# ChristophReich1996/Multi-StyleGAN

Hardware: AMD Instinct MI355X
Metric: training images/sec (G+D step, 256^2, seq=3x2ch) (higher is better)
Workload: dtype bf16

## Files before the change

multi_stylegan_amd/csrc/conv_dispatch.h:

```cpp
#pragma once
#include "msg_common.h"

struct ConvProblem {
    int dtype;
    int split;
    int B, IH, IW, Cx, Ck, OH, OW, N, ldy;
    int kh, kw, stride, pad, in_up, pixel_shuffle;
    long long w_batch_stride;

    bool per_sample() const { return w_batch_stride != 0; }
    int samples() const { return per_sample() ? B : 1; }
    long long mtot() const { return per_sample() ? (long long)OH * OW : (long long)B * OH * OW; }
    int esz() const { return dtype == MSG_BF16 ? 2 : 4; }
    long long x_bstride() const { return (long long)IH * IW * Cx; }
    long long y_bstride() const { return (pixel_shuffle ? 4ll : 1ll) * OH * OW * ldy; }
    long long x_bytes() const { return (long long)(per_sample() ? 1 : B) * IH * IW * Cx * esz(); }
    long long w_bytes() const { return (long long)N * kh * kw * Ck * esz(); }
    bool fits31() const { return x_bytes() < 0x7ffffff0ll && w_bytes() < 0x7ffffff0ll; }
};

enum ConvKernel {
    CONV_THIN_N, CONV_THIN_K,
    CONV_UPCONV,
    CONV_ROW3, CONV_ROW3N,
    CONV_PP,
    CONV_DMA, CONV_REG, CONV_REG_LEAN, CONV_REG_SPLIT
};

struct ConvPlan {
    ConvKernel kernel;
    int tile_m, tile_n;
    bool supported;
};

inline int conv_act_mode(const ActEpilogue* act) { return act ? act->enabled : 0; }

template <typename P>
inline void conv_fill_common(P& p, const ConvProblem& q, const ActEpilogue* act) {
    p.B = q.B; p.IH = q.IH; p.IW = q.IW; p.Cx = q.Cx; p.Ck = q.Ck; p.OH = q.OH; p.OW = q.OW; p.N = q.N; p.ldy = q.ldy;
    p.per_sample = q.per_sample();
    if (act) p.act = *act;
    p.x_bstride = q.x_bstride();
    p.w_bstride = q.w_batch_stride;
    p.y_bstride = q.y_bstride();
    p.Mtot = (int)q.mtot();
}
template <typename P>
inline void conv_fill_taps(P& p, const ConvProblem& q) {
    p.kh = q.kh; p.kw = q.kw; p.stride = q.stride; p.pad = q.pad; p.in_up = q.in_up; p.pixel_shuffle = q.pixel_shuffle;
}

ConvPlan conv_fprop_select(const ConvProblem& q, const ActEpilogue* act, bool has_bias);

bool conv_thin_eligible(const ConvProblem& q, const ActEpilogue* act, ConvPlan* plan);
void conv_thin_launch(const ConvProblem& q, const ConvPlan& plan, const void* x, const void* w, const float* bias, void* y,
                      const ActEpilogue* act, void* stream);
bool conv_upconv_eligible(const ConvProblem& q, const ActEpilogue* act, bool has_bias, ConvPlan* plan);
void conv_upconv_launch(const ConvProblem& q, const ConvPlan& plan, const void* x, const void* w, void* y, void* stream);
bool conv_row3_eligible(const ConvProblem& q, const ActEpilogue* act, bool has_bias, ConvPlan* plan);
void conv_row3_launch(const ConvProblem& q, const ConvPlan& plan, const void* x, const void* w, const float* bias, void* y,
                      const ActEpilogue* act, void* stream);
bool conv_pp_eligible(const ConvProblem& q, ConvPlan* plan);
void conv_pp_launch(const ConvProblem& q, const ConvPlan& plan, const void* x, const void* w, const float* bias, void* y,
                    const ActEpilogue* act, void* stream);

struct WgradProblem {
    int dtype;
    int split;
    int B, IH, IW, Cx, I, OH, OW, ldgy, O, ldgw;
    int kh, kw, stride, pad, pixel_shuffle;
    int per_sample, k_chunks, oi_major;
    float gain;
};

int conv_wgrad_row3_try(const WgradProblem& q, const void* gy, const void* x, float* gw, float* ws, long long ws_floats,
                        int plan_only, long long* need, void* stream);
extern "C" int msg_wgrad_reduce_launch(const float* ws, float* gw, long long slab, int n_out, int chunks, int O, int taps,
                                       int I, int ldgw, int oi_major, void* stream);
```

multi_stylegan_amd/csrc/conv_fprop.hip:

```cpp
#include "conv_dispatch.h"
#include <stdlib.h>

typedef __bf16 bf16v8 __attribute__((ext_vector_type(8)));
typedef const __attribute__((address_space(1))) char* gptr_t;
typedef const __attribute__((address_space(1))) u32x4* gvec_t;
typedef __attribute__((address_space(3))) char* lds_t;

struct ConvParams {
    int B, IH, IW, Cx, Ck, OH, OW, N, ldy;
    int kh, kw, stride, pad, in_up, pixel_shuffle, per_sample;
    long long x_bstride, w_bstride, y_bstride;
    int Mtot, n_chunks, n_iters, m_tiles, n_tiles;
    ActEpilogue act;
};

constexpr int BM = 128, BN = 128, ROWB = 128;
constexpr int STAGE_BYTES = (BM + BN) * ROWB;
__device__ __attribute__((aligned(256))) unsigned int g_zero_page[16384];

__device__ __forceinline__ int swz(int row, int slot) { return row * ROWB + ((slot ^ ((row >> 1) & 7)) << 4); }

template <int SPLIT>
__device__ __forceinline__ void split_park(const u32x4& raw, char* dst) {
    uint2 pl[3];
#pragma unroll
    for (int h = 0; h < 2; ++h) {
        const float x0 = __uint_as_float(raw[2 * h]), x1 = __uint_as_float(raw[2 * h + 1]);
        const unsigned hp = (unsigned)f2bf(x0) | ((unsigned)f2bf(x1) << 16);
        const float r0 = x0 - __uint_as_float(hp << 16), r1 = x1 - __uint_as_float(hp & 0xffff0000u);
        const unsigned mp = (unsigned)f2bf(r0) | ((unsigned)f2bf(r1) << 16);
        (h ? pl[0].y : pl[0].x) = hp;
        (h ? pl[1].y : pl[1].x) = mp;
        if constexpr (SPLIT == 3) {
            const float q0 = r0 - __uint_as_float(mp << 16), q1 = r1 - __uint_as_float(mp & 0xffff0000u);
            (h ? pl[2].y : pl[2].x) = (unsigned)f2bf(q0) | ((unsigned)f2bf(q1) << 16);
        }
    }
#pragma unroll
    for (int p = 0; p < SPLIT; ++p) *reinterpret_cast<uint2*>(dst + p * 64) = pl[p];
}

template <typename T, bool DMA, int LEAN = 0, int SPLIT = 0>
__global__ __launch_bounds__(256, LEAN ? LEAN : 2) void conv_fprop_kernel(const T* __restrict__ x, const T* __restrict__ w,
                                                            T* __restrict__ y, const float* __restrict__ bias,
                                                            ConvParams p) {
    constexpr int VEC = 16 / sizeof(T);
    constexpr int BKE = ROWB / sizeof(T);
    static_assert(!LEAN || (!DMA && sizeof(T) == 2), "lean variant: bf16, register staging");
    static_assert(SPLIT == 0 || sizeof(T) == 4, "split-bf16 products are a mode of the fp32-storage kernel");
    static_assert(SPLIT == 0 || !DMA, "the split planes are written from the staging registers");
    constexpr int SROW = SPLIT ? SPLIT * 64 + 16 : ROWB;
    constexpr int STAGE = SPLIT ? (BM + BN) * SROW : STAGE_BYTES;
    constexpr bool ONE_STAGE = LEAN != 0 || SPLIT == 3;
    constexpr int SMEM_BYTES = ONE_STAGE ? (STAGE > 65536 || sizeof(T) == 2 ? STAGE : 65536) : 2 * STAGE;
    __shared__ __attribute__((aligned(16))) char smem[SMEM_BYTES];

    const int tid = threadIdx.x, lane = tid & 63, wid = tid >> 6;
    const int wm = wid >> 1, wn = wid & 1;
    const int lr = lane & 31, lh = lane >> 5;
    const unsigned L = xcd_remap(blockIdx.x, gridDim.x);
    const int n0 = (int)(L % p.n_tiles) * BN;
    const int m0 = (int)(L / p.n_tiles) * BM;
    const int bz = blockIdx.z;

    const int wid_u = __builtin_amdgcn_readfirstlane(wid);
    const int slot_phys = tid & 7;
    int row_of[4];
#pragma unroll
    for (int j = 0; j < 4; ++j) row_of[j] = DMA ? (wid * 32 + 8 * j + (lane >> 3)) : ((tid >> 3) + 32 * j);
    const int slot = DMA ? 0 : slot_phys;
    int a_ih0[4], a_iw0[4];
    long long a_boff[4];
    int a_slot[4];
    bool a_ok[4];
    const int ohw = p.OH * p.OW;
#pragma unroll
    for (int j = 0; j < 4; ++j) {
        const int m = m0 + row_of[j];
        const int slot_j = DMA ? (slot_phys ^ ((row_of[j] >> 1) & 7)) : slot_phys;
        a_ok[j] = m < p.Mtot;
        const int mm = a_ok[j] ? m : 0;
        const int b = p.per_sample ? bz : mm / ohw;
        const int pix = p.per_sample ? mm : mm - b * ohw;
        const int oh = pix / p.OW, ow = pix - oh * p.OW;
        a_ih0[j] = oh * p.stride - p.pad;
        a_iw0[j] = ow * p.stride - p.pad;
        a_boff[j] = ((long long)((DMA && p.per_sample) ? 0 : b) * p.x_bstride + slot_j * VEC +
                     ((long long)a_ih0[j] * p.IW + a_iw0[j]) * p.Cx) * (long long)sizeof(T);
        a_slot[j] = slot_j;
    }
    const int taps = p.kh * p.kw;
    const gptr_t xbase = (gptr_t)x;
    const gptr_t zbase = (gptr_t)g_zero_page;
    const long long zoff = slot_phys * 16;
    gptr_t pa[4];
    gptr_t pb[4];
    {
        const gptr_t wb = (gptr_t)w + (p.per_sample ? (long long)bz * p.w_bstride : 0) * (long long)sizeof(T);
#pragma unroll
        for (int j = 0; j < 4; ++j) {
            const int n = n0 + row_of[j];
            const bool ok = n < p.N;
            pb[j] = (ok ? wb : zbase) + (ok ? ((long long)n * taps * p.Ck + a_slot[j] * VEC) * (long long)sizeof(T) : zoff);
            pa[j] = zbase;
        }
    }
    msg_desc_t d_x = {0, 0, 0, 0}, d_w = {0, 0, 0, 0};
    unsigned lds0 = 0;
    int va[4] = {MSG_DMA_OOB, MSG_DMA_OOB, MSG_DMA_OOB, MSG_DMA_OOB}, vb[4] = {MSG_DMA_OOB, MSG_DMA_OOB, MSG_DMA_OOB, MSG_DMA_OOB};
    if constexpr (DMA) {
        d_x = msg_make_desc((const char*)x + (p.per_sample ? (long long)bz * p.x_bstride * (long long)sizeof(T) : 0));
        d_w = msg_make_desc((const char*)w + (p.per_sample ? (long long)bz * p.w_bstride * (long long)sizeof(T) : 0));
        lds0 = (unsigned)(unsigned long long)(lds_t)smem;
#pragma unroll
        for (int j = 0; j < 4; ++j) {
            const int n = n0 + row_of[j];
            vb[j] = n < p.N ? (int)(((long long)n * taps * p.Ck + a_slot[j] * VEC) * (long long)sizeof(T)) : MSG_DMA_OOB;
        }
    }
    const bool ragged = (p.Cx % BKE) != 0;
    int ld_tap = -1, ld_chunk = p.n_chunks - 1;
    int kh_ = 0, kw_ = -1;
    int st_off[4];
#pragma unroll
    for (int j = 0; j < 4; ++j) st_off[j] = swz(row_of[j], a_slot[j]);

    f32x16 acc[2][2];
#pragma unroll
    for (int i = 0; i < 2; ++i)
#pragma unroll
        for (int j = 0; j < 2; ++j)
#pragma unroll
            for (int e = 0; e < 16; ++e) acc[i][j][e] = 0.f;

    u32x4 ra[4], rb[4];
    int dma_stage = 0;
    auto load_next = [&]() __attribute__((always_inline)) {
        if (++ld_chunk == p.n_chunks) {
            ld_chunk = 0;
            ++ld_tap;
            if (++kw_ == p.kw) { kw_ = 0; ++kh_; }
            if (p.in_up == 1) {
                const long long tap_off = ((long long)kh_ * p.IW + kw_) * p.Cx * (long long)sizeof(T);
#pragma unroll
                for (int j = 0; j < 4; ++j) {
                    const bool ok = a_ok[j] & ((unsigned)(a_ih0[j] + kh_) < (unsigned)p.IH) &
                                    ((unsigned)(a_iw0[j] + kw_) < (unsigned)p.IW);
                    pa[j] = (ok ? xbase : zbase) + (ok ? a_boff[j] + tap_off : zoff);
                    if constexpr (DMA) va[j] = ok ? (int)(a_boff[j] + tap_off) : MSG_DMA_OOB;
                }
            } else {
#pragma unroll
                for (int j = 0; j < 4; ++j) {
                    const int ih = a_ih0[j] + kh_, iw = a_iw0[j] + kw_;
                    bool ok = a_ok[j] & (ih >= 0) & (iw >= 0) & (ih % p.in_up == 0) & (iw % p.in_up == 0);
                    const int ihs = ih / p.in_up, iws = iw / p.in_up;
                    ok = ok & (ihs < p.IH) & (iws < p.IW);
                    const long long off = a_boff[j] + ((long long)(ihs - a_ih0[j]) * p.IW + (iws - a_iw0[j])) * p.Cx * (long long)sizeof(T);
                    pa[j] = (ok ? xbase : zbase) + (ok ? off : zoff);
                    if constexpr (DMA) va[j] = ok ? (int)off : MSG_DMA_OOB;
                }
            }
        }
#pragma unroll
        for (int j = 0; j < 4; ++j) {
            const bool c_bad = ragged && (ld_chunk * BKE + a_slot[j] * VEC + VEC > p.Cx);
            gptr_t a_addr = pa[j];
            if (c_bad) a_addr = zbase + zoff;
            if constexpr (DMA) {
                const unsigned la = lds0 + dma_stage * STAGE + (wid_u * 32 + 8 * j) * ROWB;
                msg_dma16(d_x, la, c_bad ? MSG_DMA_OOB : va[j], ld_chunk * ROWB);
                msg_dma16(d_w, la + BM * ROWB, vb[j], (ld_tap * p.n_chunks + ld_chunk) * ROWB);
            } else {
                ra[j] = *(gvec_t)a_addr;
                rb[j] = *(gvec_t)pb[j];
            }
            pa[j] += ROWB;
            pb[j] += ROWB;
        }
    };
    auto park = [&](int stage) __attribute__((always_inline)) {
        char* sa = smem + stage * STAGE;
        if constexpr (SPLIT != 0) {
            char* sb = sa + BM * SROW;
#pragma unroll
            for (int j = 0; j < 4; ++j) {
                split_park<SPLIT>(ra[j], sa + row_of[j] * SROW + slot_phys * 8);
                split_park<SPLIT>(rb[j], sb + row_of[j] * SROW + slot_phys * 8);
            }
            return;
        }
        char* sb = sa + BM * ROWB;
#pragma unroll
        for (int j = 0; j < 4; ++j) {
            *reinterpret_cast<u32x4*>(sa + st_off[j]) = ra[j];
            *reinterpret_cast<u32x4*>(sb + st_off[j]) = rb[j];
        }
    };
    auto mma_step = [&](const char* sa) __attribute__((always_inline)) {
        const char* sb = sa + BM * ROWB;
        if constexpr (sizeof(T) == 2) {
            bf16v8 fa[2][2], fb[2][2];
#pragma unroll
            for (int t = 0; t < 2; ++t) {
                fa[0][t] = *reinterpret_cast<const bf16v8*>(sa + swz(wm * 64 + t * 32 + lr, lh));
                fb[0][t] = *reinterpret_cast<const bf16v8*>(sb + swz(wn * 64 + t * 32 + lr, lh));
            }
#pragma unroll
            for (int kk = 0; kk < 4; ++kk) {
                if (kk + 1 < 4) {
#pragma unroll
                    for (int t = 0; t < 2; ++t) {
                        fa[(kk + 1) & 1][t] = *reinterpret_cast<const bf16v8*>(sa + swz(wm * 64 + t * 32 + lr, 2 * (kk + 1) + lh));
                        fb[(kk + 1) & 1][t] = *reinterpret_cast<const bf16v8*>(sb + swz(wn * 64 + t * 32 + lr, 2 * (kk + 1) + lh));
                    }
                }
#pragma unroll
                for (int i = 0; i < 2; ++i)
#pragma unroll
                    for (int j = 0; j < 2; ++j)
                        acc[i][j] = __builtin_amdgcn_mfma_f32_32x32x16_bf16(fb[kk & 1][j], fa[kk & 1][i], acc[i][j], 0, 0, 0);
            }
            __builtin_amdgcn_sched_group_barrier(0x100, 8, 0);
            __builtin_amdgcn_sched_group_barrier(0x008, 4, 0);
            __builtin_amdgcn_sched_group_barrier(0x100, 4, 0);
            __builtin_amdgcn_sched_group_barrier(0x008, 4, 0);
            __builtin_amdgcn_sched_group_barrier(0x100, 4, 0);
            __builtin_amdgcn_sched_group_barrier(0x008, 8, 0);
        } else if constexpr (SPLIT != 0) {
            const char* sbs = sa + BM * SROW;
#pragma unroll
            for (int sstep = 0; sstep < 2; ++sstep) {
                bf16v8 af[SPLIT][2], bf[SPLIT][2];
#pragma unroll
                for (int t = 0; t < 2; ++t)
#pragma unroll
                    for (int pl = 0; pl < SPLIT; ++pl) {
                        af[pl][t] = *reinterpret_cast<const bf16v8*>(sa + (wm * 64 + t * 32 + lr) * SROW + pl * 64 + (2 * sstep + lh) * 16);
                        bf[pl][t] = *reinterpret_cast<const bf16v8*>(sbs + (wn * 64 + t * 32 + lr) * SROW + pl * 64 + (2 * sstep + lh) * 16);
                    }
#pragma unroll
                for (int i = 0; i < 2; ++i)
#pragma unroll
                    for (int j = 0; j < 2; ++j) {
#pragma unroll
                        for (int order = SPLIT - 1; order >= 0; --order)
#pragma unroll
                            for (int pa = 0; pa <= order; ++pa)
                                acc[i][j] = __builtin_amdgcn_mfma_f32_32x32x16_bf16(bf[order - pa][j], af[pa][i], acc[i][j], 0, 0, 0);
                    }
            }
        } else {
#pragma unroll
            for (int q = 0; q < 4; ++q) {
                f32x4 fa[2], fb[2];
#pragma unroll
                for (int t = 0; t < 2; ++t) {
                    fa[t] = *reinterpret_cast<const f32x4*>(sa + swz(wm * 64 + t * 32 + lr, 4 * lh + q));
                    fb[t] = *reinterpret_cast<const f32x4*>(sb + swz(wn * 64 + t * 32 + lr, 4 * lh + q));
                }
#pragma unroll
                for (int e = 0; e < 4; ++e)
#pragma unroll
                    for (int i = 0; i < 2; ++i)
#pragma unroll
                        for (int j = 0; j < 2; ++j)
                            acc[i][j] = __builtin_amdgcn_mfma_f32_32x32x2f32(fb[j][e], fa[i][e], acc[i][j], 0, 0, 0);
            }
        }
    };
    if constexpr (ONE_STAGE) {
        load_next();
        for (int it = 0; it < p.n_iters; ++it) {
            if (it) __syncthreads();
            park(0);
            if (it + 1 < p.n_iters) load_next();
            __syncthreads();
            mma_step(smem);
        }
    } else {
        if constexpr (DMA) {
            dma_stage = 0;
            load_next();
        } else {
            load_next();
            park(0);
            if (p.n_iters > 1) load_next();
        }
        for (int it = 0; it < p.n_iters; ++it) {
            if constexpr (DMA) asm volatile("s_waitcnt vmcnt(0)" ::: "memory");
            __syncthreads();
            if constexpr (DMA) {
                if (it + 1 < p.n_iters) { dma_stage = (it + 1) & 1; load_next(); }
            } else {
                if (it + 1 < p.n_iters) park((it + 1) & 1);
                if (it + 2 < p.n_iters) load_next();
            }
            mma_step(smem + (it & 1) * STAGE);
        }
    }
    if constexpr (DMA) asm volatile("s_waitcnt vmcnt(0)" ::: "memory");
    __syncthreads();

    constexpr int PITCH = 64 * sizeof(T);
    constexpr int UNITB = 4 * sizeof(T);
    char* ep = smem + wid * (64 * PITCH);
#pragma unroll
    for (int j = 0; j < 2; ++j)
#pragma unroll
        for (int g = 0; g < 4; ++g) {
            const int unit = 8 * j + 2 * g + lh;
            float bv[4] = {0.f, 0.f, 0.f, 0.f};
            if (bias) {
                const int nb = n0 + wn * 64 + 4 * unit;
#pragma unroll
                for (int e = 0; e < 4; ++e) bv[e] = nb + e < p.N ? bias[nb + e] : 0.f;
            }
#pragma unroll
            for (int i = 0; i < 2; ++i) {
                const int row = i * 32 + lr;
                char* dstl = ep + row * PITCH + ((unit ^ (row & 15)) * UNITB);
                if constexpr (sizeof(T) == 2) {
                    uint2 pk;
                    pk.x = (unsigned)f2bf(acc[i][j][4 * g + 0] + bv[0]) | ((unsigned)f2bf(acc[i][j][4 * g + 1] + bv[1]) << 16);
                    pk.y = (unsigned)f2bf(acc[i][j][4 * g + 2] + bv[2]) | ((unsigned)f2bf(acc[i][j][4 * g + 3] + bv[3]) << 16);
                    *reinterpret_cast<uint2*>(dstl) = pk;
                } else {
                    *reinterpret_cast<f32x4*>(dstl) = f32x4{acc[i][j][4 * g + 0] + bv[0], acc[i][j][4 * g + 1] + bv[1],
                                                            acc[i][j][4 * g + 2] + bv[2], acc[i][j][4 * g + 3] + bv[3]};
                }
            }
        }
    constexpr int LPR = 64 / VEC;
    constexpr int RPP = 64 / LPR;
    constexpr int NPASS = 64 / RPP;
    const int er = lane / LPR, ec = (lane % LPR) * VEC;
    const int n = n0 + wn * 64 + ec;
    int nn = n, q = 0;
    if (p.pixel_shuffle) { const int oc = p.N >> 2; q = n / oc; nn = n - q * oc; }
    const int lim = p.pixel_shuffle ? (p.N >> 2) - nn : p.N - n;
    const bool n_ok = n < p.N;
    int gp[NPASS];
    float a_bias[VEC], a_noise[NPASS];
    {
        const int m_first = min(m0 + wm * 64 + er, p.Mtot - 1);
        int b = p.per_sample ? bz : m_first / ohw;
        const int pix0 = p.per_sample ? m_first : m_first - b * ohw;
        int oh = pix0 / p.OW, ow = pix0 - oh * p.OW;
        const bool want_noise = p.act.enabled == 1 && p.act.noise;
        const float nw = want_noise ? p.act.noise_w[0] : 0.f;
        if (p.act.enabled == 1) {
#pragma unroll
            for (int e = 0; e < VEC; ++e) a_bias[e] = (p.act.bias && n + e < p.N) ? p.act.bias[n + e] : 0.f;
        }
#pragma unroll
        for (int pass = 0; pass < NPASS; ++pass) {
            const bool ok = m0 + wm * 64 + pass * RPP + er < p.Mtot;
            const int pix = oh * p.OW + ow;
            const int g = p.pixel_shuffle ? ((b * 2 * p.OH + 2 * oh + (q >> 1)) * (2 * p.OW) + 2 * ow + (q & 1))
                                          : b * ohw + pix;
            gp[pass] = ok ? g : -1;
            a_noise[pass] = (want_noise && ok) ? nw * p.act.noise[(long long)(p.act.noise_batch == 1 ? 0 : b) * ohw + pix] : 0.f;
            ow += RPP;
            while (ow >= p.OW) { ow -= p.OW; ++oh; }
            if (!p.per_sample) while (oh >= p.OH) { oh -= p.OH; ++b; }
        }
    }
    __syncthreads();
    u32x4 v[NPASS];
#pragma unroll
    for (int pass = 0; pass < NPASS; ++pass) {
        const int row = pass * RPP + er;
        if constexpr (sizeof(T) == 2)
            v[pass] = *reinterpret_cast<const u32x4*>(ep + row * PITCH + (((lane & 7) ^ ((row & 15) >> 1)) << 4));
        else
            v[pass] = *reinterpret_cast<const u32x4*>(ep + row * PITCH + (((lane & 15) ^ (row & 15)) << 4));
    }
    if constexpr (sizeof(T) == 2) {
        if (er & 1) {
#pragma unroll
            for (int pass = 0; pass < NPASS; ++pass) v[pass] = u32x4{v[pass][2], v[pass][3], v[pass][0], v[pass][1]};
        }
    }
    if (p.act.enabled == 1) {
#pragma unroll
        for (int pass = 0; pass < NPASS; ++pass) v[pass] = act_epilogue_apply<T>(v[pass], a_bias, a_noise[pass], p.act.alpha, p.act.scale);
    } else if (p.act.enabled == 2) {
        const T* rbase = reinterpret_cast<const T*>(p.act.residual) + (n_ok ? n : 0);
        u32x4 r[NPASS];
#pragma unroll
        for (int pass = 0; pass < NPASS; ++pass)
            r[pass] = *reinterpret_cast<const u32x4*>(rbase + (long long)max(gp[pass], 0) * p.act.res_ld);
#pragma unroll
        for (int pass = 0; pass < NPASS; ++pass) v[pass] = residual_epilogue_apply<T>(v[pass], r[pass], p.act.res_gain);
    }
    T* ybase = y + (p.pixel_shuffle ? nn : n);
    if (n_ok && lim >= VEC) {
#pragma unroll
        for (int pass = 0; pass < NPASS; ++pass)
            if (gp[pass] >= 0) *reinterpret_cast<u32x4*>(ybase + (long long)gp[pass] * p.ldy) = v[pass];
    } else if (n_ok) {
#pragma unroll
        for (int pass = 0; pass < NPASS; ++pass) {
            if (gp[pass] < 0) continue;
            T tmp[VEC];
            *reinterpret_cast<u32x4*>(tmp) = v[pass];
            T* dst = ybase + (long long)gp[pass] * p.ldy;
            for (int e = 0; e < lim; ++e) dst[e] = tmp[e];
        }
    }
}

static ConvPlan conv_generic_select(const ConvProblem& q) {
    const int n_iters = q.kh * q.kw * (q.Ck / (ROWB / q.esz()));
    static const int variant = msg_tunable("MSG_CONV_VARIANT", 0);
    const bool dma = q.fits31() && (variant == 1 || (variant == 0 && n_iters >= 8));
    static const int lean_max = msg_tunable("MSG_CONV_LEAN", 4);
    ConvPlan plan{CONV_REG, BM, BN, true};
    if (q.split) plan.kernel = CONV_REG_SPLIT;
    else if (dma) plan.kernel = CONV_DMA;
    else if (q.dtype == MSG_BF16 && n_iters <= lean_max) plan.kernel = CONV_REG_LEAN;
    const long long mtot = q.mtot(), blocks = ((mtot + BM - 1) / BM) * ((q.N + BN - 1) / BN);
    plan.supported = mtot < (1ll << 31) && blocks < (1ll << 31) &&
                     (long long)(n_iters + 1) * ROWB + 128 <= 65536;
    return plan;
}

static void conv_generic_launch(const ConvProblem& q, const ConvPlan& plan, const void* x, const void* w, const float* bias, void* y,
                                const ActEpilogue* act, void* stream) {
    ConvParams p{};
    conv_fill_common(p, q, act);
    conv_fill_taps(p, q);
    p.n_chunks = q.Ck / (ROWB / q.esz());
    p.n_iters = q.kh * q.kw * p.n_chunks;
    p.m_tiles = (int)((q.mtot() + BM - 1) / BM);
    p.n_tiles = (q.N + BN - 1) / BN;
    dim3 grid((unsigned)((long long)p.m_tiles * p.n_tiles), 1, q.samples());
#define GENERIC(T, ...) hipLaunchKernelGGL((conv_fprop_kernel<T, __VA_ARGS__>), grid, dim3(256), 0, (hipStream_t)stream, \
                                           (const T*)x, (const T*)w, (T*)y, bias, p)
    const bool bf16 = q.dtype == MSG_BF16;
    if (bf16 && plan.kernel == CONV_REG_LEAN) GENERIC(bf16_t, false, 3);
    else if (bf16 && plan.kernel == CONV_DMA) GENERIC(bf16_t, true);
    else if (bf16) GENERIC(bf16_t, false);
    else if (plan.kernel == CONV_REG_SPLIT) GENERIC(float, false, 0, 3);
    else if (plan.kernel == CONV_DMA) GENERIC(float, true);
    else GENERIC(float, false);
#undef GENERIC
}

ConvPlan conv_fprop_select(const ConvProblem& q, const ActEpilogue* act, bool has_bias) {
    ConvPlan plan;
    if (conv_thin_eligible(q, act, &plan)) return plan;
    if (conv_upconv_eligible(q, act, has_bias, &plan)) return plan;
    if (conv_row3_eligible(q, act, has_bias, &plan)) return plan;
    if (conv_pp_eligible(q, &plan)) return plan;
    return conv_generic_select(q);
}

static ConvProblem conv_problem(int dtype, int B, int IH, int IW, int Cx, int Ck, int OH, int OW, int N, int ldy,
                                int kh, int kw, int stride, int pad, int in_up, int pixel_shuffle, long long w_batch_stride) {
    const int split = dtype == MSG_F32_SPLIT ? 3 : 0;
    return ConvProblem{split ? (int)MSG_F32 : dtype, split, B, IH, IW, Cx, Ck, OH, OW, N, ldy, kh, kw, stride, pad, in_up, pixel_shuffle,
                       w_batch_stride};
}
static ConvProblem conv_query_problem(int dtype, int B, int IH, int IW, int Cx, int Ck, int OH, int OW, int N, int kh, int kw,
                                      long long w_batch_stride) {
    return conv_problem(dtype, B, IH, IW, Cx, Ck, OH, OW, N, N <= 8 ? 8 : (N + 7) / 8 * 8, kh, kw, 1, kh / 2, 1, 0, w_batch_stride);
}

extern "C" int msg_conv2d_fprop_plan(int dtype, int B, int IH, int IW, int Cx, int Ck, int OH, int OW, int N,
                                     int kh, int kw, long long w_batch_stride) {
    switch (conv_fprop_select(conv_query_problem(dtype, B, IH, IW, Cx, Ck, OH, OW, N, kh, kw, w_batch_stride), nullptr, false).kernel) {
        case CONV_THIN_N: case CONV_THIN_K: return MSG_PLAN_THIN;
        case CONV_ROW3: return MSG_PLAN_ROW3;
        case CONV_ROW3N: return MSG_PLAN_ROW3N;
        case CONV_PP: return MSG_PLAN_PP;
        case CONV_UPCONV: return MSG_PLAN_PP;
        case CONV_DMA: return MSG_PLAN_DMA;
        default: return MSG_PLAN_REG;
    }
}

static int conv2d_fprop_impl(const void* x, const void* w, const float* bias, void* y, const ConvProblem& q,
                             const ActEpilogue& act, void* stream, const ConvPlan* selected = nullptr);

extern "C" int msg_conv2d_fprop(const void* x, const void* w, const float* bias, void* y, int dtype,
                                int B, int IH, int IW, int Cx, int Ck, int OH, int OW, int N, int ldy,
                                int kh, int kw, int stride, int pad, int in_up, int pixel_shuffle,
                                long long w_batch_stride, void* stream) {
    ActEpilogue act{};
    return conv2d_fprop_impl(x, w, bias, y, conv_problem(dtype, B, IH, IW, Cx, Ck, OH, OW, N, ldy, kh, kw, stride, pad, in_up,
                                                         pixel_shuffle, w_batch_stride), act, stream);
}

static bool is_row3(const ConvPlan& plan) { return plan.kernel == CONV_ROW3 || plan.kernel == CONV_ROW3N; }

extern "C" int msg_conv2d_fprop_act_mask(const void* x, const void* w, void* y, int dtype,
                                         int B, int IH, int IW, int Cx, int Ck, int OH, int OW, int N, int ldy,
                                         int kh, int kw, int stride, int pad, long long w_batch_stride,
                                         const float* act_bias, const float* noise, const float* noise_weight,
                                         int noise_batch, float alpha, float scale, unsigned char* mask, void* stream) {
    if (noise && (!noise_weight || (noise_batch != 1 && noise_batch != B))) return MSG_EINVAL;
    const ConvProblem q = conv_problem(dtype, B, IH, IW, Cx, Ck, OH, OW, N, ldy, kh, kw, stride, pad, 1, 0, w_batch_stride);
    ActEpilogue act{act_bias, noise, noise_weight, noise_batch, 1, alpha, scale, nullptr, 0, 0.f, mask};
    if (!mask) return conv2d_fprop_impl(x, w, nullptr, y, q, act, stream);
    const ConvPlan plan = conv_fprop_select(q, &act, false);
    return is_row3(plan) ? conv2d_fprop_impl(x, w, nullptr, y, q, act, stream, &plan) : (int)MSG_EUNSUPPORTED;
}

extern "C" int msg_conv2d_fprop_act(const void* x, const void* w, void* y, int dtype,
                                    int B, int IH, int IW, int Cx, int Ck, int OH, int OW, int N, int ldy,
                                    int kh, int kw, int stride, int pad, long long w_batch_stride,
                                    const float* act_bias, const float* noise, const float* noise_weight,
                                    int noise_batch, float alpha, float scale, void* stream) {
    return msg_conv2d_fprop_act_mask(x, w, y, dtype, B, IH, IW, Cx, Ck, OH, OW, N, ldy, kh, kw, stride, pad, w_batch_stride,
                                     act_bias, noise, noise_weight, noise_batch, alpha, scale, nullptr, stream);
}

extern "C" int msg_conv2d_fprop_residual(const void* x, const void* w, void* y, int dtype,
                                         int B, int IH, int IW, int Cx, int Ck, int OH, int OW, int N, int ldy,
                                         int kh, int kw, int stride, int pad, long long w_batch_stride,
                                         const void* residual, int res_ld, float gain, void* stream) {
    if (!residual || res_ld < N || (((uintptr_t)residual) & 15u) || res_ld % (dtype == MSG_BF16 ? 8 : 4)) return MSG_EINVAL;
    ActEpilogue act{};
    act.enabled = 2; act.residual = residual; act.res_ld = res_ld; act.res_gain = gain;
    return conv2d_fprop_impl(x, w, nullptr, y, conv_problem(dtype, B, IH, IW, Cx, Ck, OH, OW, N, ldy, kh, kw, stride, pad, 1, 0,
                                                            w_batch_stride), act, stream);
}

static void act_backward_partials(const ConvProblem& q, const ConvPlan& plan, long long* rows, long long* entries) {
    *rows = *entries = 0;
    if (!is_row3(plan)) return;
    const long long tiles = (q.mtot() / plan.tile_m) * q.samples();
    *rows = tiles * 2;
    *entries = tiles * (q.N / plan.tile_n) * 4;
}

extern "C" long long msg_conv2d_fprop_act_backward_workspace(int dtype, int B, int IH, int IW, int Cx, int Ck, int OH, int OW,
                                                             int N, int kh, int kw, long long w_batch_stride, int has_noise) {
    const ConvProblem q = conv_query_problem(dtype, B, IH, IW, Cx, Ck, OH, OW, N, kh, kw, w_batch_stride);
    ActEpilogue act{};
    act.enabled = 3;
    long long rows, entries;
    act_backward_partials(q, conv_fprop_select(q, &act, false), &rows, &entries);
    return rows ? rows * N + (has_noise ? entries : 0) : 0;
}

extern "C" int msg_conv2d_fprop_act_backward(const void* x, const void* w, void* y, int dtype,
                                             int B, int IH, int IW, int Cx, int Ck, int OH, int OW, int N, int ldy,
                                             int kh, int kw, int stride, int pad, long long w_batch_stride,
                                             const void* residual, int res_ld,
                                             const unsigned char* sign_mask, int mask_tile_m, int mask_tile_n,
                                             const void* sign_map, int sign_ld, float alpha, float scale,
                                             float* grad_bias, const float* noise, int noise_batch, float* grad_noise_weight,
                                             float* ws, long long ws_floats, void* stream) {
    if (B == 0) return MSG_OK;
    if (!x || !w || !y || B < 0) return MSG_EINVAL;
    if (!sign_mask == !sign_map) return MSG_EINVAL;
    if (stride != 1 || pad != 1 || kh != 3 || kw != 3 || ldy != N) return MSG_EUNSUPPORTED;
    const ConvProblem q = conv_problem(dtype, B, IH, IW, Cx, Ck, OH, OW, N, ldy, kh, kw, stride, pad, 1, 0, w_batch_stride);
    ActEpilogue act{};
    act.enabled = 3; act.alpha = alpha; act.scale = scale;
    const ConvPlan plan = conv_fprop_select(q, &act, false);
    long long rows, entries;
    act_backward_partials(q, plan, &rows, &entries);
    if (!rows) return MSG_EUNSUPPORTED;
    if (sign_mask && (mask_tile_m <= 0 || mask_tile_n <= 0 || mask_tile_n % 128 || N % mask_tile_n || (((uintptr_t)sign_mask) & 15u) ||
                      (mask_tile_m != 1 && mask_tile_m % 64) || ((long long)B * OH * OW) % mask_tile_m))
        return MSG_EINVAL;
    if (sign_map && (sign_ld < N || sign_ld % 8 || (((uintptr_t)sign_map) & 15u))) return MSG_EINVAL;
    if (residual && (res_ld < N || res_ld % 8 || (((uintptr_t)residual) & 15u))) return MSG_EINVAL;
    const bool has_noise = noise && grad_noise_weight;
    if (has_noise && noise_batch != 1 && noise_batch != B) return MSG_EINVAL;
    const long long need_b = grad_bias ? rows * N : 0, need_n = has_noise ? entries : 0;
    if (need_b + need_n > 0 && (!ws || ws_floats < need_b + need_n)) return MSG_EINVAL;
    act.residual = residual; act.res_ld = res_ld; act.res_gain = 1.f;
    act.mask = const_cast<unsigned char*>(sign_mask); act.mask_tile_m = mask_tile_m; act.mask_tile_n = mask_tile_n;
    act.sign_src = sign_map; act.sign_ld = sign_ld;
    act.noise = has_noise ? noise : nullptr; act.noise_batch = noise_batch;
    act.part_b = grad_bias ? ws : nullptr;
    act.part_n = has_noise ? ws + need_b : nullptr;
    conv_row3_launch(q, plan, x, w, nullptr, y, &act, stream);
    if (MSG_CHECK_LAUNCH() != MSG_OK) return MSG_ELAUNCH;
    return msg_bias_act_reduce_launch(act.part_b, grad_bias, N, rows, act.part_n, grad_noise_weight, entries, stream);
}

static int conv2d_fprop_impl(const void* x, const void* w, const float* bias, void* y, const ConvProblem& q,
                             const ActEpilogue& act, void* stream, const ConvPlan* selected) {
    if (q.B == 0) return MSG_OK;
    if (!x || !w || !y || q.B < 0 || q.IH <= 0 || q.IW <= 0 || q.OH <= 0 || q.OW <= 0 || q.N <= 0 || q.kh <= 0 || q.kw <= 0 ||
        q.stride <= 0 || q.in_up <= 0 || q.Cx <= 0 || q.Ck <= 0 || q.ldy <= 0)
        return MSG_EINVAL;
    if (q.dtype != MSG_F32 && q.dtype != MSG_BF16) return MSG_EUNSUPPORTED;
    const int vec = 16 / q.esz(), bke = ROWB / q.esz();
    if (q.Ck % bke || q.Cx % vec || (((uintptr_t)x | (uintptr_t)w | (uintptr_t)y) & 15u)) return MSG_EUNSUPPORTED;
    if (q.ldy % vec || (q.pixel_shuffle && (q.N % 4 || (q.N / 4) % vec))) return MSG_EUNSUPPORTED;
    if (q.in_up > 1 && q.stride != 1) return MSG_EUNSUPPORTED;
    const ConvPlan plan = selected ? *selected : conv_fprop_select(q, &act, bias != nullptr);
    if (!plan.supported) return MSG_EUNSUPPORTED;
    switch (plan.kernel) {
        case CONV_THIN_N: case CONV_THIN_K: conv_thin_launch(q, plan, x, w, bias, y, &act, stream); break;
        case CONV_UPCONV: conv_upconv_launch(q, plan, x, w, y, stream); break;
        case CONV_ROW3: case CONV_ROW3N: conv_row3_launch(q, plan, x, w, bias, y, &act, stream); break;
        case CONV_PP: conv_pp_launch(q, plan, x, w, bias, y, &act, stream); break;
        case CONV_DMA: case CONV_REG: case CONV_REG_LEAN: case CONV_REG_SPLIT:
            conv_generic_launch(q, plan, x, w, bias, y, &act, stream); break;
    }
    return MSG_CHECK_LAUNCH();
}
```

Measured before the change: 156.5.

## Add persistent streaming 1x1 conv kernel with LDS-resident weights and DMA ring

Adds a persistent bf16 kernel for large 1x1 convolutions with Ck of 128 or 256. Each block keeps its weight slice in LDS and streams activation tiles through a per-wave six-slot DMA ring, using counted vmcnt waits. This lets the next tiles load while MFMA and the epilogue run, and avoids re-reading weights for every output tile as the generic tiled kernel does. The grid is sized to the CU count, and the path is gated by a minimum tile count and restricted activation modes. The hand-counted waits are fragile and can break correctness if the load or store counts drift.

New measurement: 156.9, median of 6. No clear change (+0.3%).

```diff
diff --git a/multi_stylegan_amd/csrc/conv_dispatch.h b/multi_stylegan_amd/csrc/conv_dispatch.h
--- a/multi_stylegan_amd/csrc/conv_dispatch.h
+++ b/multi_stylegan_amd/csrc/conv_dispatch.h
@@ -24,6 +24,7 @@
     CONV_UPCONV,
     CONV_ROW3, CONV_ROW3N,
     CONV_PP,
+    CONV_REG_STREAM,
     CONV_DMA, CONV_REG, CONV_REG_LEAN, CONV_REG_SPLIT
 };
 
@@ -63,6 +64,9 @@
 bool conv_pp_eligible(const ConvProblem& q, ConvPlan* plan);
 void conv_pp_launch(const ConvProblem& q, const ConvPlan& plan, const void* x, const void* w, const float* bias, void* y,
                     const ActEpilogue* act, void* stream);
+bool conv_stream_eligible(const ConvProblem& q, const ActEpilogue* act, ConvPlan* plan);
+void conv_stream_launch(const ConvProblem& q, const ConvPlan& plan, const void* x, const void* w, const float* bias, void* y,
+                        const ActEpilogue* act, void* stream);
 
 struct WgradProblem {
     int dtype;
diff --git a/multi_stylegan_amd/csrc/conv_fprop.hip b/multi_stylegan_amd/csrc/conv_fprop.hip
--- a/multi_stylegan_amd/csrc/conv_fprop.hip
+++ b/multi_stylegan_amd/csrc/conv_fprop.hip
@@ -454,6 +454,7 @@
     if (conv_upconv_eligible(q, act, has_bias, &plan)) return plan;
     if (conv_row3_eligible(q, act, has_bias, &plan)) return plan;
     if (conv_pp_eligible(q, &plan)) return plan;
+    if (conv_stream_eligible(q, act, &plan)) return plan;
     return conv_generic_select(q);
 }
 
@@ -603,6 +604,7 @@
         case CONV_UPCONV: conv_upconv_launch(q, plan, x, w, y, stream); break;
         case CONV_ROW3: case CONV_ROW3N: conv_row3_launch(q, plan, x, w, bias, y, &act, stream); break;
         case CONV_PP: conv_pp_launch(q, plan, x, w, bias, y, &act, stream); break;
+        case CONV_REG_STREAM: conv_stream_launch(q, plan, x, w, bias, y, &act, stream); break;
         case CONV_DMA: case CONV_REG: case CONV_REG_LEAN: case CONV_REG_SPLIT:
             conv_generic_launch(q, plan, x, w, bias, y, &act, stream); break;
     }
diff --git a/multi_stylegan_amd/csrc/conv_fprop_stream.hip b/multi_stylegan_amd/csrc/conv_fprop_stream.hip
--- /dev/null
+++ b/multi_stylegan_amd/csrc/conv_fprop_stream.hip
@@ -0,0 +1,263 @@
+#include "conv_dispatch.h"
+
+typedef __bf16 bf16v8 __attribute__((ext_vector_type(8)));
+typedef __attribute__((address_space(3))) char* lds_t;
+
+struct StreamParams {
+    int Mtot, Cx, N, ldy, m_tiles;
+    ActEpilogue act;
+};
+
+constexpr int ST_RING = 6;
+constexpr int ST_MAX_N_K128 = 512;
+constexpr int ST_SLOT = 32 * 128;
+constexpr int ST_MIN_TILES = 4096;
+
+template <int N> __device__ __forceinline__ void st_wait_vm() {
+    asm volatile("s_waitcnt vmcnt(%0)" ::"n"(N < 63 ? N : 63) : "memory");
+}
+
+template <int KC, int NT>
+__global__ __launch_bounds__(256, 1) void conv_fprop_stream_kernel(const bf16_t* __restrict__ x, const bf16_t* __restrict__ w,
+                                                                   bf16_t* __restrict__ y, const float* __restrict__ bias,
+                                                                   StreamParams p) {
+    constexpr int NR = 128 * NT;
+    constexpr int NJ = 4 * NT;
+    constexpr int NH = 2 * NT;
+    constexpr int W_BYTES = NR * KC * 128;
+    static_assert(KC == 2 || KC == 4, "the counted waits below are written for these two");
+    __shared__ __attribute__((aligned(16))) char smem[W_BYTES + 4 * ST_RING * ST_SLOT];
+
+    const int tid = threadIdx.x, lane = tid & 63;
+    const int wid = __builtin_amdgcn_readfirstlane(tid >> 6);
+    const int lr = lane & 31, lh = lane >> 5;
+    const int ns0 = blockIdx.y * NR;
+    const int G = gridDim.x, bid = blockIdx.x;
+    const int n_my = (p.m_tiles - bid + G - 1) / G;
+    const bool res = p.act.enabled == 2;
+
+    const msg_desc_t d_x = msg_make_desc(x);
+    const unsigned ring0 = (unsigned)(unsigned long long)(lds_t)smem + W_BYTES + wid * (ST_RING * ST_SLOT);
+    char* const ring = smem + W_BYTES + wid * (ST_RING * ST_SLOT);
+
+    const int drow = lane >> 3, dphys = lane & 7;
+    auto issue = [&](int tile, int k, int slot) __attribute__((always_inline)) {
+        const int mw = tile * 128 + wid * 32;
+#pragma unroll
+        for (int i = 0; i < 4; ++i) {
+            const int r = 8 * i + drow, m = mw + r;
+            const bool ok = tile < p.m_tiles && m < p.Mtot;
+            const int voff = ok ? (int)(((long long)m * p.Cx + ((dphys ^ ((r >> 1) & 7)) << 3)) * 2) : MSG_DMA_OOB;
+            msg_dma16(d_x, ring0 + slot * ST_SLOT + i * 1024, voff, k * 128);
+        }
+    };
+
+    int i_tile = bid, i_k = 0, i_slot = 0;
+    auto issue_next = [&]() __attribute__((always_inline)) {
+        issue(i_tile, i_k, i_slot);
+        if (++i_k == KC) { i_k = 0; i_tile += G; }
+        if (++i_slot == ST_RING) i_slot = 0;
+    };
+#pragma unroll
+    for (int c = 0; c < ST_RING; ++c) issue_next();
+    for (int idx = tid; idx < NR * KC * 8; idx += 256) {
+        const int slot = idx & 7, r = (idx >> 3) % NR, k = idx / (8 * NR);
+        const int n = ns0 + r;
+        u32x4 v = {0u, 0u, 0u, 0u};
+        if (n < p.N) v = *reinterpret_cast<const u32x4*>(w + (long long)n * (KC * 64) + k * 64 + slot * 8);
+        *reinterpret_cast<u32x4*>(smem + (k * NR + r) * 128 + ((slot ^ ((r >> 1) & 7)) << 4)) = v;
+    }
+    asm volatile("s_waitcnt vmcnt(0)" ::: "memory");
+    __syncthreads();
+
+    const int er = lane >> 3, ec = lane & 7;
+    float a_bias[NH][8];
+#pragma unroll
+    for (int h = 0; h < NH; ++h)
+#pragma unroll
+        for (int e = 0; e < 8; ++e) a_bias[h][e] = 0.f;
+    if (p.act.enabled == 1 && p.act.bias) {
+#pragma unroll
+        for (int h = 0; h < NH; ++h)
+#pragma unroll
+            for (int e = 0; e < 8; ++e) a_bias[h][e] = p.act.bias[ns0 + 64 * h + ec * 8 + e];
+    }
+    asm volatile("s_waitcnt vmcnt(0)" ::: "memory");
+
+    const int sw = (lr >> 1) & 7;
+    const char* const wl = smem + lr * 128;
+    int c_slot = 0;
+    for (int it = 0; it < n_my; ++it) {
+        const int tile = bid + it * G;
+        const int mw = tile * 128 + wid * 32;
+        const bool full = mw + 32 <= p.Mtot;
+        const int t_slot = c_slot;
+
+        u32x4 rv[NH][4];
+        if (res) {
+#pragma unroll
+            for (int h = 0; h < NH; ++h)
+#pragma unroll
+                for (int pass = 0; pass < 4; ++pass) {
+                    const int m = min(mw + pass * 8 + er, p.Mtot - 1);
+                    rv[h][pass] = *reinterpret_cast<const u32x4*>(reinterpret_cast<const bf16_t*>(p.act.residual) +
+                                                                  (long long)m * p.act.res_ld + ns0 + 64 * h + ec * 8);
+                }
+        }
+
+        f32x16 acc[NJ];
+#pragma unroll
+        for (int j = 0; j < NJ; ++j)
+#pragma unroll
+            for (int e = 0; e < 16; ++e) acc[j][e] = 0.f;
+
+#pragma unroll
+        for (int k = 0; k < KC; ++k) {
+#ifdef MSG_STREAM_NO_STORE_COUNT
+            constexpr int S = 0, R = 4 * NH;
+#else
+            constexpr int S = 4 * NH, R = 4 * NH;
+#endif
+            if constexpr (KC == 4) {
+                if (res) { if (k == 0) st_wait_vm<20 + 2 * (S + R)>(); else if (k == 1) st_wait_vm<16 + 2 * (S + R)>(); else if (k == 2) st_wait_vm<12 + S + R>(); else st_wait_vm<8 + S + R>(); }
+                else     { if (k == 0) st_wait_vm<20 + 2 * S>(); else if (k == 1) st_wait_vm<16 + 2 * S>(); else if (k == 2) st_wait_vm<12 + S>(); else st_wait_vm<8 + S>(); }
+            } else {
+                if (res) { if (k == 0) st_wait_vm<20 + 3 * (S + R)>(); else st_wait_vm<16 + 3 * (S + R)>(); }
+                else     { if (k == 0) st_wait_vm<20 + 3 * S>(); else st_wait_vm<16 + 3 * S>(); }
+            }
+            const char* sa = ring + c_slot * ST_SLOT + lr * 128;
+            const char* sb = wl + k * (NR * 128);
+#pragma unroll
+            for (int kk = 0; kk < 4; ++kk) {
+                const int off = ((2 * kk + lh) ^ sw) << 4;
+                const bf16v8 fa = *reinterpret_cast<const bf16v8*>(sa + off);
+#pragma unroll
+                for (int j = 0; j < NJ; ++j) {
+                    const bf16v8 fb = *reinterpret_cast<const bf16v8*>(sb + j * (32 * 128) + off);
+                    acc[j] = __builtin_amdgcn_mfma_f32_32x32x16_bf16(fb, fa, acc[j], 0, 0, 0);
+                }
+            }
+            if (++c_slot == ST_RING) c_slot = 0;
+        }
+
+        asm volatile("s_waitcnt lgkmcnt(0)" ::: "memory");
+        u32x4 v[NH][4];
+#pragma unroll
+        for (int h = 0; h < NH; ++h) {
+            int ps = t_slot + (h % KC);
+            if (ps >= ST_RING) ps -= ST_RING;
+            char* patch = ring + ps * ST_SLOT;
+#pragma unroll
+            for (int jj = 0; jj < 2; ++jj)
+#pragma unroll
+                for (int g = 0; g < 4; ++g) {
+                    const int j = 2 * h + jj;
+                    float bv[4] = {0.f, 0.f, 0.f, 0.f};
+                    if (bias) {
+                        const float* bp = bias + ns0 + 32 * j + 8 * g;
+#pragma unroll
+                        for (int e = 0; e < 4; ++e) {
+                            const int lo = __builtin_amdgcn_readfirstlane(__float_as_int(bp[e]));
+                            const int hi = __builtin_amdgcn_readfirstlane(__float_as_int(bp[4 + e]));
+                            bv[e] = __int_as_float(lh ? hi : lo);
+                        }
+                    }
+                    uint2 pk;
+                    pk.x = (unsigned)f2bf(acc[j][4 * g + 0] + bv[0]) | ((unsigned)f2bf(acc[j][4 * g + 1] + bv[1]) << 16);
+                    pk.y = (unsigned)f2bf(acc[j][4 * g + 2] + bv[2]) | ((unsigned)f2bf(acc[j][4 * g + 3] + bv[3]) << 16);
+                    const int unit = 8 * jj + 2 * g + lh;
+                    *reinterpret_cast<uint2*>(patch + lr * 128 + ((unit ^ (lr & 15)) << 3)) = pk;
+                }
+            asm volatile("s_waitcnt lgkmcnt(0)" ::: "memory");
+#pragma unroll
+            for (int pass = 0; pass < 4; ++pass) {
+                const int row = pass * 8 + er;
+                v[h][pass] = *reinterpret_cast<const u32x4*>(patch + row * 128 + ((ec ^ ((row & 15) >> 1)) << 4));
+            }
+            asm volatile("s_waitcnt lgkmcnt(0)" ::: "memory");
+        }
+        if (er & 1) {
+#pragma unroll
+            for (int h = 0; h < NH; ++h)
+#pragma unroll
+                for (int pass = 0; pass < 4; ++pass) v[h][pass] = u32x4{v[h][pass][2], v[h][pass][3], v[h][pass][0], v[h][pass][1]};
+        }
+        if (p.act.enabled == 1) {
+#pragma unroll
+            for (int h = 0; h < NH; ++h)
+#pragma unroll
+                for (int pass = 0; pass < 4; ++pass)
+                    v[h][pass] = act_epilogue_apply<bf16_t>(v[h][pass], a_bias[h], 0.f, p.act.alpha, p.act.scale);
+        } else if (res) {
+#pragma unroll
+            for (int h = 0; h < NH; ++h)
+#pragma unroll
+                for (int pass = 0; pass < 4; ++pass)
+                    v[h][pass] = residual_epilogue_apply<bf16_t>(v[h][pass], rv[h][pass], p.act.res_gain);
+        }
+#pragma unroll
+        for (int h = 0; h < NH; ++h)
+#pragma unroll
+            for (int pass = 0; pass < 4; ++pass) asm volatile("" : "+v"(v[h][pass]));
+#pragma unroll
+        for (int k = 0; k < KC; ++k) issue_next();
+
+        bf16_t* yb = y + ns0 + ec * 8;
+        if (full) {
+#pragma unroll
+            for (int h = 0; h < NH; ++h)
+#pragma unroll
+                for (int pass = 0; pass < 4; ++pass)
+                    *reinterpret_cast<u32x4*>(yb + (long long)(mw + pass * 8 + er) * p.ldy + 64 * h) = v[h][pass];
+        } else {
+#pragma unroll
+            for (int h = 0; h < NH; ++h)
+#pragma unroll
+                for (int pass = 0; pass < 4; ++pass) {
+                    const int m = mw + pass * 8 + er;
+                    if (m < p.Mtot) *reinterpret_cast<u32x4*>(yb + (long long)m * p.ldy + 64 * h) = v[h][pass];
+                }
+        }
+    }
+    asm volatile("s_waitcnt vmcnt(0)" ::: "memory");
+}
+
+bool conv_stream_eligible(const ConvProblem& q, const ActEpilogue* act, ConvPlan* plan) {
+    static const int enabled = msg_tunable("MSG_CONV_STREAM", 1);
+    static const int min_tiles = msg_tunable("MSG_CONV_STREAM_MIN_TILES", ST_MIN_TILES);
+    if (!enabled || q.dtype != MSG_BF16 || q.split || q.per_sample() || q.pixel_shuffle) return false;
+    if (q.kh != 1 || q.kw != 1 || q.stride != 1 || q.pad != 0 || q.in_up != 1 || q.IH != q.OH || q.IW != q.OW) return false;
+    if (q.Cx != q.Ck || (q.Ck != 128 && q.Ck != 256) || q.N % 128) return false;
+    const int mode = conv_act_mode(act);
+    if (mode != 0 && mode != 2 && !(mode == 1 && !act->noise)) return false;
+    if (enabled != 2) {
+        const int max_n = q.Ck == 128 ? ST_MAX_N_K128 : 128;
+        if (q.N > max_n) return false;
+        if (mode == 2 && !(q.Ck == 128 && q.N % 256 == 0)) return false;
+    }
+    const long long mtot = q.mtot(), tiles = (mtot + 127) / 128;
+    if (mtot >= (1ll << 30) || q.x_bytes() >= 0x7ffffff0ll || tiles < (enabled == 2 ? 256 : min_tiles)) return false;
+    *plan = ConvPlan{CONV_REG_STREAM, 128, q.Ck == 128 && q.N % 256 == 0 ? 256 : 128, true};
+    return true;
+}
+
+void conv_stream_launch(const ConvProblem& q, const ConvPlan& plan, const void* x, const void* w, const float* bias, void* y,
+                        const ActEpilogue* act, void* stream) {
+    static const int cus = [] {
+        int dev = 0, n = 0;
+        if (hipGetDevice(&dev) != hipSuccess || hipDeviceGetAttribute(&n, hipDeviceAttributeMultiprocessorCount, dev) != hipSuccess || n <= 0)
+            n = 256;
+        return n;
+    }();
+    StreamParams p{};
+    p.Mtot = (int)q.mtot(); p.Cx = q.Cx; p.N = q.N; p.ldy = q.ldy;
+    p.m_tiles = (int)((q.mtot() + 127) / 128);
+    if (act) p.act = *act;
+    dim3 grid((unsigned)(p.m_tiles < cus ? p.m_tiles : cus), (unsigned)(q.N / plan.tile_n), 1);
+#define STREAM(KC, NT) hipLaunchKernelGGL((conv_fprop_stream_kernel<KC, NT>), grid, dim3(256), 0, (hipStream_t)stream, \
+                                          (const bf16_t*)x, (const bf16_t*)w, (bf16_t*)y, bias, p)
+    if (q.Ck == 256) STREAM(4, 1);
+    else if (plan.tile_n == 256) STREAM(2, 2);
+    else STREAM(2, 1);
+#undef STREAM
+}
```
